# ai2cm/ace

Measured on AMD Instinct MI355X. Metric: rollout steps/sec (6-hourly forward steps of the 1-degree SFNO, whole job), higher is better.
Workload: dtype f32 (contractions with K>=32 on error-compensated fp16x3 MFMA, fp32 accumulate; DFT, norms, epilogues fp32; measured error vs fp64 below the fp32 CPU reference's); 1 GPU; ACE2-ERA5-shape 1deg SFNO rollout (BASELINE.json configs[1]): embed 384, 8 layers, dhconv, 44 in / 50 out channels, 180x360 legendre-gauss, lmax 180, mmax 181, B=1 member per GPU, random-init weights; members=1, members_per_gpu=1, graph=step, precision=f16x3, collective=none

## Files before the change

### ace_amd/build.py

```python

import concurrent.futures
import os
import shutil
import subprocess

HERE = os.path.dirname(os.path.abspath(__file__))
CSRC = os.path.join(HERE, "csrc")
OBJ = os.path.join(CSRC, "build")
LIB = os.path.join(HERE, "libace_sfno.so")
SOURCES = ["kernels.hip", "fft.hip", "strip.hip", "strip_fold.hip", "conv_ws.hip", "conv_wl.hip", "dhconv_strip.hip", "cln_mfma.hip", "physics.hip", "ocean_phys.hip", "masking.hip", "diag.hip", "hist.hip", "regress.hip", "calendar.hip", "healpix.hip", "latlon.hip", "capi.hip", "tables.cpp"]
HEADERS = ["kernels.h", "strip_common.h", "strip_pack.h", "ws_plan.h", "pack_frag.h", "dhconv_units.h", "tuning_guard.h", "small_fft.h", "tables.h", "diag_common.h", os.path.join("..", "..", "include", "ace_sfno.h")]
FLAGS = ["--offload-arch=gfx950", "-O3", "-std=c++17", "-fPIC"]


def _hipcc() -> str:
    for cand in (shutil.which("hipcc"), "/opt/rocm/bin/hipcc"):
        if cand and os.path.exists(cand):
            return cand
    raise RuntimeError("hipcc not found (need ROCm >= 7.0 to build libace_sfno.so)")


def _mtime(path: str) -> float:
    return os.path.getmtime(path) if os.path.exists(path) else 0.0


def _header_time() -> float:
    return max(_mtime(os.path.join(CSRC, h)) for h in HEADERS)


def source_sha256() -> str:
    import hashlib
    h = hashlib.sha256()
    for name in sorted(SOURCES + HEADERS):
        with open(os.path.join(CSRC, name), "rb") as f:
            h.update(name.encode() + b"\0" + f.read() + b"\0")
    h.update(" ".join(FLAGS).encode())
    return h.hexdigest()


def needs_build() -> bool:
    if not os.path.exists(LIB):
        return True
    t = os.path.getmtime(LIB)
    deps = [os.path.join(CSRC, s) for s in SOURCES + HEADERS]
    return any(os.path.exists(d) and os.path.getmtime(d) > t for d in deps)


def _compile(hipcc: str, src: str, obj: str, extra, verbose: bool) -> None:
    cmd = [hipcc] + FLAGS + list(extra) + ["-c", src, "-o", obj]
    if verbose:
        print(" ".join(cmd), flush=True)
    res = subprocess.run(cmd, capture_output=True, text=True)
    if res.returncode != 0:
        raise RuntimeError(f"hipcc failed on {src}:\n" + res.stdout + res.stderr)


def build(force: bool = False, verbose: bool = False, out: str = LIB, extra=(), objdir: str = OBJ) -> str:
    if out == LIB and extra:
        raise ValueError("the shipped library is built with the default flags only; a variant (extra flags) needs its own `out` and `objdir`")
    if extra and not any(f == "-DACE_MEASUREMENT_SWITCHES" for f in extra):
        extra = list(extra) + ["-DACE_MEASUREMENT_SWITCHES"]
    if not force and out == LIB and not needs_build():
        return LIB
    hipcc = _hipcc()
    os.makedirs(objdir, exist_ok=True)
    for stale in os.listdir(objdir):
        if stale.endswith(".o") and stale[:-2] not in SOURCES:
            os.remove(os.path.join(objdir, stale))
    ht = _header_time()
    jobs, objs = [], []
    for s in SOURCES:
        src = os.path.join(CSRC, s)
        obj = os.path.join(objdir, s + ".o")
        objs.append(obj)
        if force or _mtime(obj) < max(_mtime(src), ht):
            jobs.append((src, obj))
    with concurrent.futures.ThreadPoolExecutor(max_workers=max(1, min(len(jobs), os.cpu_count() or 1))) as ex:
        for f in [ex.submit(_compile, hipcc, src, obj, extra, verbose) for src, obj in jobs]:
            f.result()
    cmd = [hipcc, "--offload-arch=gfx950", "-shared", "-fPIC", "-o", out + ".tmp"] + objs
    if verbose:
        print(" ".join(cmd), flush=True)
    res = subprocess.run(cmd, capture_output=True, text=True)
    if res.returncode != 0:
        raise RuntimeError("link failed:\n" + res.stdout + res.stderr)
    os.replace(out + ".tmp", out)
    return out


if __name__ == "__main__":
    import sys

    print(build(force="--force" in sys.argv, verbose=True))
```

### ace_amd/csrc/conv_wl.hip

```cpp
#include <hip/hip_runtime.h>

#include <cstdint>

#include "strip_common.h"

namespace ace {
namespace {

#ifndef ACE_WL_WAVES
#define ACE_WL_WAVES 8
#endif
#ifndef ACE_WL_D
#define ACE_WL_D 4
#endif
#ifndef ACE_WL_ABL
#define ACE_WL_ABL 0
#endif
constexpr int WL_WAVES = ACE_WL_WAVES;
#ifdef ACE_X_TRACE
__device__ unsigned long long wl_wg_span[4096][3];
#define WG_STAMP(k) do { if (threadIdx.x == 0 && blockIdx.x < 4096) wl_wg_span[blockIdx.x][k] = __builtin_amdgcn_s_memtime(); } while (0)
#else
#define WG_STAMP(k) do { } while (0)
#endif
constexpr int WL_OOBV = 0x7fffff00;

template <int KS, int RT, int D, bool FOLD = false>
__global__ __launch_bounds__(64 * WL_WAVES) void conv_wl_kernel(ConvStripArgs p, int nslice, int groups_per_xcd, int tpx) {
    constexpr int FTB = FOLD ? (2 * 16 * KS + WL_WAVES * 32 * RT + 16) * 4 : 0;
    __shared__ __attribute__((aligned(16))) char smem[RT * KS * 2048 + 32 * RT * 4 + FTB];
    float* Pb = reinterpret_cast<float*>(smem + RT * KS * 2048);
    const int tid = threadIdx.x;
    const int lane = tid & 63;
    const int wave = __builtin_amdgcn_readfirstlane(tid >> 6);
    const int i = lane & 31, g = lane >> 5;

    const int per_xcd = nslice * groups_per_xcd;
    const int per_smp = 8 * per_xcd;
    const int smp = blockIdx.x / per_smp;
    const int bb = blockIdx.x % per_smp;
    const int xcd = bb & 7, w = bb >> 3;
    const int slice = w % nslice, grp = w / nslice;
    const int tiles_px = (p.HW + 31) / 32;
    const int x0 = xcd * tpx;
    const int x1 = x0 + tpx < tiles_px ? x0 + tpx : tiles_px;

    MT(0);
    WG_STAMP(0);
    const unsigned raw_x = slot_load(p.xslot + lane);
    const unsigned raw_a = (!FOLD && p.aslot) ? slot_load(p.aslot + lane) : 0u;
    const unsigned raw_c = p.cinb ? slot_load(p.cinb + lane) : 0u;

    float fscale = 1.f;
    if constexpr (FOLD) {
        static_assert(WL_WAVES == 8 && KS % 8 == 0, "fold: wave w takes the k-steps w, w + 8, ... of every row tile");
        float* Ta = Pb + 32 * RT;
        float* Tb = Ta + 16 * KS;
        float* Pd = Tb + 16 * KS;
        float* red = Pd + WL_WAVES * 32 * RT;
        const float* fa = p.fa + (long)smp * p.sfa;
        const float* fb = p.fb + (long)smp * p.sfa;
        float am = 0.f;
        for (int r = tid; r < 16 * KS; r += 64 * WL_WAVES) {
            const float av = fa[r];
            Ta[r] = av; Tb[r] = fb[r];
            am = fmaxf(am, fabsf(av));
        }
#pragma unroll
        for (int off = 32; off > 0; off >>= 1) am = fmaxf(am, __shfl_xor(am, off, 64));
        if (lane == 0) red[wave] = am;
        __syncthreads();
        am = red[0];
#pragma unroll
        for (int k = 1; k < WL_WAVES; ++k) am = fmaxf(am, red[k]);
        fscale = ldexpf(1.0f, pow2_exponent_for(p.wabs * am));
#pragma unroll
        for (int t = 0; t < RT; ++t) {
            const float* Wr = p.Wraw + (long)(32 * (slice * RT + t) + i) * p.ldw + 8 * g;
            float dot = 0.f;
#pragma unroll
            for (int jj = 0; jj < KS / 8; ++jj) {
                const int J = wave + 8 * jj;
                const f32x4 w0 = *reinterpret_cast<const f32x4*>(Wr + 16 * J), w1 = *reinterpret_cast<const f32x4*>(Wr + 16 * J + 4);
                const int col = 16 * J + 8 * g;
                const f32x4 a0 = *reinterpret_cast<const f32x4*>(Ta + col), a1 = *reinterpret_cast<const f32x4*>(Ta + col + 4);
                const f32x4 b0 = *reinterpret_cast<const f32x4*>(Tb + col), b1 = *reinterpret_cast<const f32x4*>(Tb + col + 4);
                half8 fh, fl;
#pragma unroll
                for (int e = 0; e < 8; ++e) {
                    const float wv = e < 4 ? w0[e & 3] : w1[e & 3];
                    dot = fmaf(wv, e < 4 ? b0[e & 3] : b1[e & 3], dot);
                    float x = wv * fscale;
                    x *= e < 4 ? a0[e & 3] : a1[e & 3];
                    x = __builtin_amdgcn_fmed3f(x, -65504.f, 65504.f);
                    const _Float16 hv = (_Float16)x;
                    fh[e] = hv;
                    fl[e] = (_Float16)(x - (float)hv);
                }
                *reinterpret_cast<half8*>(smem + (t * KS + J) * 2048 + lane * 16) = fh;
                *reinterpret_cast<half8*>(smem + (t * KS + J) * 2048 + 1024 + lane * 16) = fl;
            }
            dot += __shfl_xor(dot, 32, 64);
            if (g == 0) Pd[wave * (32 * RT) + 32 * t + i] = dot;
        }
        __syncthreads();
        if (tid < 32 * RT) {
            float acc = Pd[tid];
#pragma unroll
            for (int k = 1; k < WL_WAVES; ++k) acc += Pd[k * (32 * RT) + tid];
            Pb[tid] = p.bias[slice * 32 * RT + tid] + acc;
        }
    } else {
        const char* A = reinterpret_cast<const char*>(p.A + (long)smp * p.sA) + (long)slice * RT * KS * 2048;
        for (int o = tid * 16; o < RT * KS * 2048; o += 64 * WL_WAVES * 16)
            *reinterpret_cast<u32x4*>(smem + o) = *reinterpret_cast<const u32x4*>(A + o);
        const float* b = p.bias + (long)smp * p.sbias + slice * 32 * RT;
        if (tid < 32 * RT) Pb[tid] = b[tid];
    }
    const float xbound = wave_max_bits(raw_x);
    const float inv_x = ldexpf(1.0f, -pow2_exponent_for(xbound));
    const float inv_a = FOLD ? 1.0f / fscale : (p.aslot ? ldexpf(1.0f, -pow2_exponent_for(wave_max_bits(raw_a))) : 1.0f / p.ascale);
    const float s_acc = inv_x * inv_a;
    const float inb = p.cinb ? wave_max_bits(raw_c) : xbound;
    const float cbound = fmaf(p.cw, inb, p.cb);
    const float cscale = ldexpf(1.0f, pow2_exponent_for(cbound));
    if (tid == 0) atomicMax(p.cslot + (blockIdx.x & 63), __float_as_uint(cbound));
    __syncthreads();
    MT(1);
    int tev = 2;

    const _Float16* Xh = p.Xhi + (long)smp * p.sX;
    const _Float16* Xl = p.Xlo + (long)smp * p.sX;
    const int pbytes = p.M * p.HW * 2;
    const int xbytes = p.C * (int)p.ldn * 2;
    const auto rsXh = __builtin_amdgcn_make_buffer_rsrc(const_cast<_Float16*>(Xh), 0, xbytes, 0x00020000);
    const auto rsXl = __builtin_amdgcn_make_buffer_rsrc(const_cast<_Float16*>(Xl), 0, xbytes, 0x00020000);
    const auto rsH = __builtin_amdgcn_make_buffer_rsrc(p.Chi + (long)smp * p.sCp, 0, pbytes, 0x00020000);
    const auto rsL = __builtin_amdgcn_make_buffer_rsrc(p.Clo + (long)smp * p.sCp, 0, pbytes, 0x00020000);
    const char* aw = smem + lane * 16;

    f32x16 prev[RT];
#pragma unroll
    for (int t = 0; t < RT; ++t)
#pragma unroll
        for (int r = 0; r < 16; ++r) prev[t][r] = 0.f;
    int prev_vo = WL_OOBV;
    GeluStage gst = {0.f, 0.f, 0.f};
    unsigned hh[4] = {0u, 0u, 0u, 0u}, ll[4] = {0u, 0u, 0u, 0u};
    float bias_next = Pb[8 * g];
    auto chunk = [&](auto kc) {
        constexpr int k = decltype(kc)::value;
        constexpr int v = k / 4, ch = k % 4, t = v / 16, q = (v % 16) / 8, e = v % 8;
        if constexpr (ch == 0) {
            gelu_stage0(gst, fmaf(prev[t][8 * q + e], s_acc, bias_next));
            asm volatile("" : "+v"(gst.val), "+v"(gst.t));
        } else if constexpr (ch == 1) {
            gelu_stage1(gst);
            constexpr int vn = (v + 1) % (16 * RT);
            bias_next = Pb[32 * (vn / 16) + 16 * ((vn % 16) / 8) + 8 * g + vn % 8];
            asm volatile("" : "+v"(gst.q));
        } else if constexpr (ch == 2) {
            gst.val = gelu_stage2(gst);
            asm volatile("" : "+v"(gst.val));
        } else {
            split_put<e>(hh, ll, cscale, gst.val);
            if constexpr (e == 7) {
                const int soff = (4 * (slice * RT + t) + 2 * q) * p.HW * 16;
                __builtin_amdgcn_raw_buffer_store_b128(u32x4{hh[0], hh[1], hh[2], hh[3]}, rsH, prev_vo, soff, 0);
                __builtin_amdgcn_raw_buffer_store_b128(u32x4{ll[0], ll[1], ll[2], ll[3]}, rsL, prev_vo, soff, 0);
            }
        }
    };
    constexpr int NCH = 4 * 16 * RT;
    constexpr int NM = 9 * KS;
    static_assert(RT == 3 || RT == 2, "slot arithmetic below");
    constexpr int MPS = 3 * RT;
    auto slot = [&](auto mc) {
        constexpr int m = decltype(mc)::value;
        constexpr int NMT = MPS * KS;
        if constexpr (!(ACE_WL_ABL & 1)) static_for<(m * NCH) / NMT, ((m + 1) * NCH) / NMT>([&](auto kc) { chunk(kc); });
        __builtin_amdgcn_sched_barrier(0);
    };
    (void)NM;

    const int stride = WL_WAVES * groups_per_xcd;
    for (int tile = x0 + grp * WL_WAVES + wave; tile < x1; tile += stride) {
        MT(tev);
        int n = 32 * tile + i;
        const bool nok = n < p.HW;
        n = nok ? n : p.HW - 1;
        const int bvo = (g * (int)p.ldn + n) * 16;
        const int kstep = 2 * (int)p.ldn * 16;
        f32x16 acc[RT];
#pragma unroll
        for (int t = 0; t < RT; ++t)
#pragma unroll
            for (int r = 0; r < 16; ++r) acc[t][r] = 0.f;
        half8 bh[D], bl[D];
#pragma unroll
        for (int d = 0; d < D; ++d) {
            bh[d] = __builtin_bit_cast(half8, __builtin_amdgcn_raw_buffer_load_b128(rsXh, bvo, d * kstep, 0));
            bl[d] = __builtin_bit_cast(half8, __builtin_amdgcn_raw_buffer_load_b128(rsXl, bvo, d * kstep, 0));
        }
        half8 ah[2][RT], al[2][RT];
#pragma unroll
        for (int t = 0; t < RT; ++t) {
            ah[0][t] = *reinterpret_cast<const half8*>(aw + (t * KS) * 2048);
            al[0][t] = *reinterpret_cast<const half8*>(aw + (t * KS) * 2048 + 1024);
        }
        static_for<0, KS>([&](auto jc) {
            constexpr int j = decltype(jc)::value;
            const half8 ch = bh[j % D], cl = bl[j % D];
            if constexpr (j + 1 < KS) {
#pragma unroll
                for (int t = 0; t < RT; ++t) {
                    ah[(j + 1) & 1][t] = *reinterpret_cast<const half8*>(aw + (t * KS + j + 1) * 2048);
                    al[(j + 1) & 1][t] = *reinterpret_cast<const half8*>(aw + (t * KS + j + 1) * 2048 + 1024);
                }
            }
            __builtin_amdgcn_sched_barrier(0);
            static_for<0, RT>([&](auto tc) {
                constexpr int t = decltype(tc)::value;
                acc[t] = __builtin_amdgcn_mfma_f32_32x32x16_f16(al[j & 1][t], ch, acc[t], 0, 0, 0);
                slot(std::integral_constant<int, MPS * j + t>{});
            });
            static_for<0, RT>([&](auto tc) {
                constexpr int t = decltype(tc)::value;
                acc[t] = __builtin_amdgcn_mfma_f32_32x32x16_f16(ah[j & 1][t], cl, acc[t], 0, 0, 0);
                slot(std::integral_constant<int, MPS * j + RT + t>{});
            });
            static_for<0, RT>([&](auto tc) {
                constexpr int t = decltype(tc)::value;
                acc[t] = __builtin_amdgcn_mfma_f32_32x32x16_f16(ah[j & 1][t], ch, acc[t], 0, 0, 0);
                if constexpr (t == RT - 1 && j + D < KS && !(ACE_WL_ABL & 2)) {
                    bh[j % D] = __builtin_bit_cast(half8, __builtin_amdgcn_raw_buffer_load_b128(rsXh, bvo, (j + D) * kstep, 0));
                    bl[j % D] = __builtin_bit_cast(half8, __builtin_amdgcn_raw_buffer_load_b128(rsXl, bvo, (j + D) * kstep, 0));
                }
                slot(std::integral_constant<int, MPS * j + 2 * RT + t>{});
            });
        });
        MT(tev + 1);
        tev += 2;
#pragma unroll
        for (int t = 0; t < RT; ++t) {
            rows_to_kgroups(acc[t]);
            prev[t] = acc[t];
        }
        prev_vo = nok ? ((g * p.HW + 32 * tile + i) * 16) : WL_OOBV;
    }
    static_for<0, NCH>([&](auto kc) { chunk(kc); });
    MT(tev);
    WG_STAMP(1);
#ifdef ACE_X_TRACE
    if (threadIdx.x == 0 && blockIdx.x < 4096) {
        unsigned xcc;
        asm volatile("s_getreg_b32 %0, hwreg(HW_REG_XCC_ID)" : "=s"(xcc));
        wl_wg_span[blockIdx.x][2] = xcc & 0xf;
    }
#endif
}

template <int KS, int RT, int D, bool FOLD = false>
hipError_t launch_wl(const ConvStripArgs& a, hipStream_t s) {
    const int nslice = a.M / (32 * RT);
    int gpx = 32 / nslice;
    if (gpx < 1) gpx = 1;
    const int tiles_px = (int)((a.HW + 31) / 32);
    const int tpx = (tiles_px + 7) / 8;
    if (gpx * WL_WAVES > tpx) gpx = (tpx + WL_WAVES - 1) / WL_WAVES;
    dim3 grid((unsigned)(8 * nslice * gpx * a.nbatch)), block(64 * WL_WAVES);
    hipLaunchKernelGGL((conv_wl_kernel<KS, RT, D, FOLD>), grid, block, 0, s, a, nslice, gpx, tpx);
    return hipGetLastError();
}

}

#ifdef ACE_X_TRACE
extern "C" int ace_debug_trace(void* dst) { return (int)hipMemcpyFromSymbol(dst, HIP_SYMBOL(mlp_trace), sizeof(mlp_trace)); }
extern "C" int ace_debug_wg_spans(void* dst) { return (int)hipMemcpyFromSymbol(dst, HIP_SYMBOL(wl_wg_span), sizeof(wl_wg_span)); }
#endif

bool conv_wl_eligible(int K, int M, long HW) {
    if (K == 384) return M % 96 == 0 && M / 96 <= 32 && (long)M * HW * 2 < 0x7fffff00L;
    if (K == 512 || K == 256 || K == 128) return M % 64 == 0 && M / 64 <= 32 && (long)M * HW * 2 < 0x7fffff00L;
    return false;
}

hipError_t launch_conv_wl(const ConvStripArgs& a, hipStream_t s) {
    if (!conv_wl_eligible(a.C, a.M, a.HW) || !a.bias || !a.xslot || !(a.A || a.Wraw) || !a.Chi || !a.Clo || !a.cslot || a.R || a.part || a.Cf ||
        !(a.act == ACT_GELU || a.act == ACT_GELU_FAST))
        return hipErrorInvalidValue;
    if (a.Wraw) {
        if (!a.fa || !a.fb || (a.ldw & 3) != 0 || (reinterpret_cast<uintptr_t>(a.Wraw) & 15) != 0 || a.sbias != 0 || a.C != 384) return hipErrorInvalidValue;
        return launch_wl<24, 3, ACE_WL_D, true>(a, s);
    }
    switch (a.C) {
        case 512: return launch_wl<32, 2, 4>(a, s);
        case 384: return launch_wl<24, 3, ACE_WL_D>(a, s);
        case 256: return launch_wl<16, 2, 4>(a, s);
        case 128: return launch_wl<8, 2, 4>(a, s);
        default: return hipErrorInvalidValue;
    }
}

}
```

### ace_amd/csrc/strip_common.h

```cpp
#pragma once
#include <hip/hip_runtime.h>

#include <type_traits>

#include "kernels.h"

namespace ace {
namespace {

#define MDEV __device__ __forceinline__
#ifndef ACE_MLP_FDEPTH
#define ACE_MLP_FDEPTH 2
#endif
#ifndef ACE_MLP_ABL
#define ACE_MLP_ABL 0
#endif

typedef _Float16 half8 __attribute__((ext_vector_type(8)));
typedef float f32x16 __attribute__((ext_vector_type(16)));
typedef float f32x4 __attribute__((ext_vector_type(4)));
typedef unsigned u32x4 __attribute__((ext_vector_type(4)));
typedef __attribute__((address_space(3))) char* lds_cptr;

MDEV unsigned slot_load(const unsigned* p) { return __hip_atomic_load(p, __ATOMIC_RELAXED, __HIP_MEMORY_SCOPE_AGENT); }
MDEV int pow2_exponent_for(float mx) {
    int e = 0;
    if (mx > 0.f && mx < 3.0e38f) { (void)frexpf(mx, &e); e = 12 - e; }
    return e > 100 ? 100 : (e < -100 ? -100 : e);
}
MDEV float wave_max_bits(unsigned raw) {
    float mx = __uint_as_float(raw);
#pragma unroll
    for (int off = 32; off > 0; off >>= 1) mx = fmaxf(mx, __shfl_xor(mx, off, 64));
    return __uint_as_float(__builtin_amdgcn_readfirstlane(__float_as_uint(mx)));
}
MDEV void glds16(const void* gsrc, const char* lds_dst_uniform) {
    const unsigned addr = __builtin_amdgcn_readfirstlane((unsigned)(size_t)(lds_cptr)lds_dst_uniform);
    asm volatile("s_mov_b32 m0, %1\n\ts_nop 0\n\tglobal_load_lds_dwordx4 %0, off"
                 :
                 : "v"(gsrc), "s"(addr)
                 : "memory", "m0");
}
MDEV void glds16s(const void* sbase_uniform, unsigned lane_off, const char* lds_dst_uniform) {
    const unsigned addr = __builtin_amdgcn_readfirstlane((unsigned)(size_t)(lds_cptr)lds_dst_uniform);
    asm volatile("s_mov_b32 m0, %2\n\ts_nop 0\n\tglobal_load_lds_dwordx4 %0, %1"
                 :
                 : "v"(lane_off), "s"(sbase_uniform), "s"(addr)
                 : "memory", "m0");
}
MDEV unsigned lds_addr_of(const char* p) { return __builtin_amdgcn_readfirstlane((unsigned)(size_t)(lds_cptr)p); }
MDEV void glds16a(const void* sbase_uniform, unsigned lane_off, unsigned lds_addr_uniform) {
    asm volatile("s_mov_b32 m0, %2\n\ts_nop 0\n\tglobal_load_lds_dwordx4 %0, %1"
                 :
                 : "v"(lane_off), "s"(sbase_uniform), "s"(lds_addr_uniform)
                 : "memory", "m0");
}
MDEV float fast_erf(float x) {
    const float t = fminf(fabsf(x), 4.0f);
    float q = -1.150086973e-05f;
    q = fmaf(q, t, 1.518900972e-04f);
    q = fmaf(q, t, -8.436889620e-04f);
    q = fmaf(q, t, 2.264559502e-03f);
    q = fmaf(q, t, -7.151089812e-05f);
    q = fmaf(q, t, -2.773463540e-02f);
    q = fmaf(q, t, 1.483123451e-01f);
    q = fmaf(q, t, 9.184418917e-01f);
    q = fmaf(q, t, 1.627907395e+00f);
    q = q * t;
    return copysignf(1.0f - __builtin_amdgcn_exp2f(-q), x);
}
struct GeluStage { float val, t, q; };
MDEV void gelu_stage0(GeluStage& g, float val) {
    g.val = val;
    g.t = fminf(fabsf(val), 5.65685424949238f);
}
MDEV void gelu_stage1(GeluStage& g) {
    float q = -5.082714551e-07f;
    q = fmaf(q, g.t, 9.493131074e-06f);
    q = fmaf(q, g.t, -7.457227184e-05f);
    q = fmaf(q, g.t, 2.830699377e-04f);
    q = fmaf(q, g.t, -1.264146067e-05f);
    q = fmaf(q, g.t, -6.933658849e-03f);
    q = fmaf(q, g.t, 5.243633315e-02f);
    q = fmaf(q, g.t, 4.592209458e-01f);
    q = fmaf(q, g.t, 1.151104331e+00f);
    g.q = q;
}
MDEV float gelu_stage2(const GeluStage& g) {
    const float q = g.q * g.t;
    const float s = g.val + fabsf(g.val);
    return 0.5f * fmaf(-g.t, __builtin_amdgcn_exp2f(-q), s);
}

template <int E>
MDEV void split_put(unsigned (&H)[4], unsigned (&L)[4], const float cs, const float v) {
    constexpr int d = E >> 1;
    if constexpr ((E & 1) == 0) {
        asm volatile("v_fma_mixlo_f16 %0, %2, %3, 0\n\tv_fma_mixlo_f16 %1, %2, %3, -%0 op_sel_hi:[0,0,1]" : "+v"(H[d]), "+v"(L[d]) : "v"(cs), "v"(v));
    } else {
        unsigned tmp;
        asm volatile("v_fma_mixlo_f16 %2, %3, %4, 0\n\tv_fma_mixhi_f16 %0, %3, %4, 0\n\tv_fma_mixhi_f16 %1, %3, %4, -%2 op_sel_hi:[0,0,1]"
                     : "+v"(H[d]), "+v"(L[d]), "=&v"(tmp)
                     : "v"(cs), "v"(v));
    }
}

template <int ACT>
MDEV float act_fn(float v) {
    if (ACT == ACT_GELU_FAST || ACT == ACT_GELU) { GeluStage g; gelu_stage0(g, v); gelu_stage1(g); return gelu_stage2(g); }
    if (ACT == ACT_RELU) return v > 0.f ? v : 0.f;
    if (ACT == ACT_SILU) return v / (1.0f + expf(-v));
    return v;
}

MDEV void rows_to_kgroups(f32x16& v) {
#pragma unroll
    for (int hq = 0; hq < 2; ++hq)
#pragma unroll
        for (int e = 0; e < 4; ++e) {
            const auto sw = __builtin_amdgcn_permlane32_swap(__float_as_uint(v[8 * hq + e]), __float_as_uint(v[8 * hq + 4 + e]), false, false);
            v[8 * hq + e] = __uint_as_float(sw[0]);
            v[8 * hq + 4 + e] = __uint_as_float(sw[1]);
        }
}

#ifdef ACE_X_TRACE
__device__ unsigned long long mlp_trace[512];
#define MT(ev) do { if (blockIdx.x == ACE_X_TRACE && threadIdx.x == 0 && (ev) < 512) mlp_trace[ev] = __builtin_amdgcn_s_memtime(); } while (0)
#else
#define MT(ev) do { } while (0)
#endif

template <int I0, int I1, class F>
MDEV void static_for(F&& f);

struct Frag { half8 h, l; };
template <int OFF>
MDEV void frag_issue(Frag& f, unsigned lds_addr) {
    asm volatile("ds_read_b128 %0, %2 offset:%3\n\tds_read_b128 %1, %2 offset:%4"
                 : "=&v"(f.h), "=&v"(f.l)
                 : "v"(lds_addr), "n"(OFF), "n"(OFF + 1024));
}
template <int N>
MDEV void frag_wait(Frag& f) {
    asm volatile("s_waitcnt lgkmcnt(%2)" : "+v"(f.h), "+v"(f.l) : "n"(N));
}
template <int NS, int DEPTH, class F>
MDEV void pipelined_steps(unsigned lds_addr, F&& body) {
    Frag fr[DEPTH + 1];
    static_for<0, (DEPTH < NS ? DEPTH : NS)>([&](auto ss) {
        constexpr int s0 = decltype(ss)::value;
        frag_issue<s0 * 2048>(fr[s0 % (DEPTH + 1)], lds_addr);
    });
    static_for<0, NS>([&](auto ss) {
        constexpr int st = decltype(ss)::value;
        if constexpr (st + DEPTH < NS) frag_issue<(st + DEPTH) * 2048>(fr[(st + DEPTH) % (DEPTH + 1)], lds_addr);
        constexpr int newer = (NS - 1 - st) < DEPTH ? (NS - 1 - st) : DEPTH;
        frag_wait<2 * newer>(fr[st % (DEPTH + 1)]);
        body(ss, fr[st % (DEPTH + 1)]);
    });
}

template <int NS, class F>
MDEV void pipelined_pairs(unsigned lds_addr, F&& body) {
    static_assert(NS % 2 == 0, "units of two k-steps");
    constexpr int NU = NS / 2;
    Frag fr[2][2];
#if ACE_MLP_ABL & 2
    for (int a = 0; a < 2; ++a) for (int b = 0; b < 2; ++b) { asm volatile("" : "=v"(fr[a][b].h), "=v"(fr[a][b].l)); }
    static_for<0, NU>([&](auto uu) { constexpr int u = decltype(uu)::value; body(uu, fr[u % 2][0], fr[u % 2][1]); });
    return;
#endif
    frag_issue<0>(fr[0][0], lds_addr);
    frag_issue<2048>(fr[0][1], lds_addr);
    static_for<0, NU>([&](auto uu) {
        constexpr int u = decltype(uu)::value;
        if constexpr (u + 1 < NU) {
            frag_issue<(2 * u + 2) * 2048>(fr[(u + 1) % 2][0], lds_addr);
            frag_issue<(2 * u + 3) * 2048>(fr[(u + 1) % 2][1], lds_addr);
        }
        constexpr int newer = u + 1 < NU ? 4 : 0;
        asm volatile("s_waitcnt lgkmcnt(%4)"
                     : "+v"(fr[u % 2][0].h), "+v"(fr[u % 2][0].l), "+v"(fr[u % 2][1].h), "+v"(fr[u % 2][1].l)
                     : "n"(newer));
        body(uu, fr[u % 2][0], fr[u % 2][1]);
    });
}

template <int I0, int I1, class F>
MDEV void static_for(F&& f) {
    if constexpr (I0 < I1) {
        f(std::integral_constant<int, I0>{});
        static_for<I0 + 1, I1>(f);
    }
}


}
}
```

### ace_amd/csrc/tuning_guard.h

```cpp
#pragma once
#if !defined(ACE_MEASUREMENT_SWITCHES)
#if defined(ACE_WL_ABL) || defined(ACE_WL_D) || defined(ACE_WL_WAVES) || defined(ACE_WS_ABL) || defined(ACE_WS_ACC2) || defined(ACE_WS_FD4) || \
    defined(ACE_WS_FINE) || defined(ACE_WS_HOLD4) || defined(ACE_WS_VSPAN) || defined(ACE_WS_REARLY) || defined(ACE_WS_MINMAX) || defined(ACE_FFT_ABL) || defined(ACE_FFT_FWD_WAVES) || defined(ACE_FFT_FWD_PLN_WAVES) ||            \
    defined(ACE_FFT_INV_ROWS) || defined(ACE_FFT_INV_WAVES) || defined(ACE_FFT_QROWS) || defined(ACE_FFT_ROWS) || defined(ACE_FFT_XCD) ||       \
    defined(ACE_FFT_XCD_INV) || defined(ACE_G4_PIN) || defined(ACE_EXP_NOLDSREAD) || defined(ACE_EXP_NOBARRIER) || defined(ACE_EXP_NOGLOBAL) || \
    defined(ACE_EXP_NOLDSWRITE) || defined(ACE_G3_W128_PCT) || defined(ACE_G4_PFD) || defined(ACE_G4_REGEPI) || defined(ACE_G4_RTOUCH) ||       \
    defined(ACE_GEMM2_BK) || defined(ACE_LB) || defined(ACE_PF) || defined(ACE_MLP_ABL) || defined(ACE_MLP_FDEPTH) || defined(ACE_X_TRACE) ||    \
    defined(ACE_DH_TRACE) || defined(ACE_DH_TRACE_WG) || defined(ACE_DH_PB) || defined(ACE_DH_WGS) || defined(ACE_DH_STRIPS) || defined(ACE_DH_ORDER) || defined(ACE_LF_TRACE) || defined(ACE_DEBUG_WS)
#error "tuning / ablation / trace macro set without -DACE_MEASUREMENT_SWITCHES: the shipped library is built with the defaults only (tools/mkvar.sh)"
#endif
#endif
```

Before: 185.7 steps/s.

## Switch conv_wl main loop from 32x32x16 to 16x16x32 MFMA tiles

Adds a default-on path in the conv_wl kernel that computes each 32x32 output tile as four 16x16 sub-tiles using the 16x16x32 f16 MFMA, with new lane/offset maps for the A reads from LDS and the B loads from global. The accumulators are permuted back into the old k-group register layout with permlane16_swap, so the epilogue stays unchanged. The aim is to use the MFMA shape with higher issue throughput or better latency hiding on gfx950. In exchange it issues four times as many MFMA instructions, changes the load pattern and register use, and adds a cross-lane shuffle per tile.

```diff
diff --git a/ace_amd/build.py b/ace_amd/build.py
--- a/ace_amd/build.py
+++ b/ace_amd/build.py
@@ -9,7 +9,7 @@
 OBJ = os.path.join(CSRC, "build")
 LIB = os.path.join(HERE, "libace_sfno.so")
 SOURCES = ["kernels.hip", "fft.hip", "strip.hip", "strip_fold.hip", "conv_ws.hip", "conv_wl.hip", "dhconv_strip.hip", "cln_mfma.hip", "physics.hip", "ocean_phys.hip", "masking.hip", "diag.hip", "hist.hip", "regress.hip", "calendar.hip", "healpix.hip", "latlon.hip", "capi.hip", "tables.cpp"]
-HEADERS = ["kernels.h", "strip_common.h", "strip_pack.h", "ws_plan.h", "pack_frag.h", "dhconv_units.h", "tuning_guard.h", "small_fft.h", "tables.h", "diag_common.h", os.path.join("..", "..", "include", "ace_sfno.h")]
+HEADERS = ["kernels.h", "strip_common.h", "mfma16_map.h", "strip_pack.h", "ws_plan.h", "pack_frag.h", "dhconv_units.h", "tuning_guard.h", "small_fft.h", "tables.h", "diag_common.h", os.path.join("..", "..", "include", "ace_sfno.h")]
 FLAGS = ["--offload-arch=gfx950", "-O3", "-std=c++17", "-fPIC"]
 
 
diff --git a/ace_amd/csrc/conv_wl.hip b/ace_amd/csrc/conv_wl.hip
--- a/ace_amd/csrc/conv_wl.hip
+++ b/ace_amd/csrc/conv_wl.hip
@@ -15,6 +15,9 @@
 #endif
 #ifndef ACE_WL_ABL
 #define ACE_WL_ABL 0
+#endif
+#ifndef ACE_WL_SHAPE16
+#define ACE_WL_SHAPE16 1
 #endif
 constexpr int WL_WAVES = ACE_WL_WAVES;
 #ifdef ACE_X_TRACE
@@ -25,7 +28,7 @@
 #endif
 constexpr int WL_OOBV = 0x7fffff00;
 
-template <int KS, int RT, int D, bool FOLD = false>
+template <int KS, int RT, int D, bool FOLD = false, bool S16 = (ACE_WL_SHAPE16 != 0)>
 __global__ __launch_bounds__(64 * WL_WAVES) void conv_wl_kernel(ConvStripArgs p, int nslice, int groups_per_xcd, int tpx) {
     constexpr int FTB = FOLD ? (2 * 16 * KS + WL_WAVES * 32 * RT + 16) * 4 : 0;
     __shared__ __attribute__((aligned(16))) char smem[RT * KS * 2048 + 32 * RT * 4 + FTB];
@@ -174,7 +177,7 @@
     constexpr int NCH = 4 * 16 * RT;
     constexpr int NM = 9 * KS;
     static_assert(RT == 3 || RT == 2, "slot arithmetic below");
-    constexpr int MPS = 3 * RT;
+    constexpr int MPS = S16 ? 6 * RT : 3 * RT;
     auto slot = [&](auto mc) {
         constexpr int m = decltype(mc)::value;
         constexpr int NMT = MPS * KS;
@@ -189,62 +192,126 @@
         int n = 32 * tile + i;
         const bool nok = n < p.HW;
         n = nok ? n : p.HW - 1;
-        const int bvo = (g * (int)p.ldn + n) * 16;
-        const int kstep = 2 * (int)p.ldn * 16;
-        f32x16 acc[RT];
-#pragma unroll
-        for (int t = 0; t < RT; ++t)
-#pragma unroll
-            for (int r = 0; r < 16; ++r) acc[t][r] = 0.f;
-        half8 bh[D], bl[D];
-#pragma unroll
-        for (int d = 0; d < D; ++d) {
-            bh[d] = __builtin_bit_cast(half8, __builtin_amdgcn_raw_buffer_load_b128(rsXh, bvo, d * kstep, 0));
-            bl[d] = __builtin_bit_cast(half8, __builtin_amdgcn_raw_buffer_load_b128(rsXl, bvo, d * kstep, 0));
-        }
-        half8 ah[2][RT], al[2][RT];
-#pragma unroll
-        for (int t = 0; t < RT; ++t) {
-            ah[0][t] = *reinterpret_cast<const half8*>(aw + (t * KS) * 2048);
-            al[0][t] = *reinterpret_cast<const half8*>(aw + (t * KS) * 2048 + 1024);
-        }
-        static_for<0, KS>([&](auto jc) {
-            constexpr int j = decltype(jc)::value;
-            const half8 ch = bh[j % D], cl = bl[j % D];
-            if constexpr (j + 1 < KS) {
-#pragma unroll
-                for (int t = 0; t < RT; ++t) {
-                    ah[(j + 1) & 1][t] = *reinterpret_cast<const half8*>(aw + (t * KS + j + 1) * 2048);
-                    al[(j + 1) & 1][t] = *reinterpret_cast<const half8*>(aw + (t * KS + j + 1) * 2048 + 1024);
+        if constexpr (S16) {
+            static_assert(D % 2 == 0 && KS % 2 == 0, "k32-steps");
+            constexpr int DJ = D / 2, NJ = KS / 2;
+            int bvo[2];
+#pragma unroll
+            for (int ph = 0; ph < 2; ++ph) {
+                int np = 32 * tile + m16::b_pixel(ph, lane);
+                np = np < p.HW ? np : p.HW - 1;
+                bvo[ph] = (m16::b_kgroup(0, lane) * (int)p.ldn + np) * 16;
+            }
+            const int kstep = m16::b_kgroup(1, 0) * (int)p.ldn * 16;
+            f32x4 acc[RT][2][2];
+#pragma unroll
+            for (int t = 0; t < RT; ++t)
+#pragma unroll
+                for (int r = 0; r < 16; ++r) acc[t][r >> 3][(r >> 2) & 1][r & 3] = 0.f;
+            half8 bh[DJ][2], bl[DJ][2];
+#pragma unroll
+            for (int d = 0; d < DJ; ++d)
+#pragma unroll
+                for (int ph = 0; ph < 2; ++ph) {
+                    bh[d][ph] = __builtin_bit_cast(half8, __builtin_amdgcn_raw_buffer_load_b128(rsXh, bvo[ph], d * kstep, 0));
+                    bl[d][ph] = __builtin_bit_cast(half8, __builtin_amdgcn_raw_buffer_load_b128(rsXl, bvo[ph], d * kstep, 0));
                 }
-            }
-            __builtin_amdgcn_sched_barrier(0);
-            static_for<0, RT>([&](auto tc) {
-                constexpr int t = decltype(tc)::value;
-                acc[t] = __builtin_amdgcn_mfma_f32_32x32x16_f16(al[j & 1][t], ch, acc[t], 0, 0, 0);
-                slot(std::integral_constant<int, MPS * j + t>{});
+            const char* aw16[2] = {smem + m16::a_lane_byte(0, lane), smem + m16::a_lane_byte(1, lane)};
+            auto a_read = [&](auto hc, half8 (&dh)[RT], half8 (&dl)[RT]) {
+                constexpr int hs = decltype(hc)::value, J = hs >> 1, a = hs & 1;
+                static_for<0, RT>([&](auto kc) {
+                    constexpr int rt = a * RT + decltype(kc)::value;
+                    const char* src = aw16[rt & 1] + m16::a_row_tile32(rt) * KS * 2048 + J * m16::A_STEP_BYTES;
+                    dh[decltype(kc)::value] = *reinterpret_cast<const half8*>(src);
+                    dl[decltype(kc)::value] = *reinterpret_cast<const half8*>(src + m16::A_LO_BYTES);
+                });
+            };
+            half8 ah[2][RT], al[2][RT];
+            a_read(std::integral_constant<int, 0>{}, ah[0], al[0]);
+            static_for<0, 2 * NJ>([&](auto hc) {
+                constexpr int hs = decltype(hc)::value, J = hs >> 1, a = hs & 1;
+                if constexpr (hs + 1 < 2 * NJ) a_read(std::integral_constant<int, hs + 1>{}, ah[(hs + 1) & 1], al[(hs + 1) & 1]);
+                __builtin_amdgcn_sched_barrier(0);
+                static_for<0, 3>([&](auto pc) {
+                    constexpr int pr = decltype(pc)::value;
+                    static_for<0, 2 * RT>([&](auto kc) {
+                        constexpr int k = decltype(kc)::value, x = k >> 1, ph = k & 1, rt = a * RT + x;
+                        const half8 av = pr == 0 ? al[hs & 1][x] : ah[hs & 1][x];
+                        const half8 bv = pr == 1 ? bl[J % DJ][ph] : bh[J % DJ][ph];
+                        acc[rt >> 1][rt & 1][ph] = __builtin_amdgcn_mfma_f32_16x16x32_f16(av, bv, acc[rt >> 1][rt & 1][ph], 0, 0, 0);
+                        if constexpr (a == 1 && pr == 2 && k == 2 * RT - 1 && J + DJ < NJ && !(ACE_WL_ABL & 2)) {
+#pragma unroll
+                            for (int q = 0; q < 2; ++q) {
+                                bh[J % DJ][q] = __builtin_bit_cast(half8, __builtin_amdgcn_raw_buffer_load_b128(rsXh, bvo[q], (J + DJ) * kstep, 0));
+                                bl[J % DJ][q] = __builtin_bit_cast(half8, __builtin_amdgcn_raw_buffer_load_b128(rsXl, bvo[q], (J + DJ) * kstep, 0));
+                            }
+                        }
+                        slot(std::integral_constant<int, MPS * hs + 2 * RT * pr + k>{});
+                    });
+                });
             });
-            static_for<0, RT>([&](auto tc) {
-                constexpr int t = decltype(tc)::value;
-                acc[t] = __builtin_amdgcn_mfma_f32_32x32x16_f16(ah[j & 1][t], cl, acc[t], 0, 0, 0);
-                slot(std::integral_constant<int, MPS * j + RT + t>{});
+            MT(tev + 1);
+            tev += 2;
+#pragma unroll
+            for (int t = 0; t < RT; ++t) prev[t] = tiles16_to_kgroups(acc[t]);
+        } else {
+            const int bvo = (g * (int)p.ldn + n) * 16;
+            const int kstep = 2 * (int)p.ldn * 16;
+            f32x16 acc[RT];
+    #pragma unroll
+            for (int t = 0; t < RT; ++t)
+    #pragma unroll
+                for (int r = 0; r < 16; ++r) acc[t][r] = 0.f;
+            half8 bh[D], bl[D];
+    #pragma unroll
+            for (int d = 0; d < D; ++d) {
+                bh[d] = __builtin_bit_cast(half8, __builtin_amdgcn_raw_buffer_load_b128(rsXh, bvo, d * kstep, 0));
+                bl[d] = __builtin_bit_cast(half8, __builtin_amdgcn_raw_buffer_load_b128(rsXl, bvo, d * kstep, 0));
+            }
+            half8 ah[2][RT], al[2][RT];
+    #pragma unroll
+            for (int t = 0; t < RT; ++t) {
+                ah[0][t] = *reinterpret_cast<const half8*>(aw + (t * KS) * 2048);
+                al[0][t] = *reinterpret_cast<const half8*>(aw + (t * KS) * 2048 + 1024);
+            }
+            static_for<0, KS>([&](auto jc) {
+                constexpr int j = decltype(jc)::value;
+                const half8 ch = bh[j % D], cl = bl[j % D];
+                if constexpr (j + 1 < KS) {
+    #pragma unroll
+                    for (int t = 0; t < RT; ++t) {
+                        ah[(j + 1) & 1][t] = *reinterpret_cast<const half8*>(aw + (t * KS + j + 1) * 2048);
+                        al[(j + 1) & 1][t] = *reinterpret_cast<const half8*>(aw + (t * KS + j + 1) * 2048 + 1024);
+                    }
+                }
+                __builtin_amdgcn_sched_barrier(0);
+                static_for<0, RT>([&](auto tc) {
+                    constexpr int t = decltype(tc)::value;
+                    acc[t] = __builtin_amdgcn_mfma_f32_32x32x16_f16(al[j & 1][t], ch, acc[t], 0, 0, 0);
+                    slot(std::integral_constant<int, MPS * j + t>{});
+                });
+                static_for<0, RT>([&](auto tc) {
+                    constexpr int t = decltype(tc)::value;
+                    acc[t] = __builtin_amdgcn_mfma_f32_32x32x16_f16(ah[j & 1][t], cl, acc[t], 0, 0, 0);
+                    slot(std::integral_constant<int, MPS * j + RT + t>{});
+                });
+                static_for<0, RT>([&](auto tc) {
+                    constexpr int t = decltype(tc)::value;
+                    acc[t] = __builtin_amdgcn_mfma_f32_32x32x16_f16(ah[j & 1][t], ch, acc[t], 0, 0, 0);
+                    if constexpr (t == RT - 1 && j + D < KS && !(ACE_WL_ABL & 2)) {
+                        bh[j % D] = __builtin_bit_cast(half8, __builtin_amdgcn_raw_buffer_load_b128(rsXh, bvo, (j + D) * kstep, 0));
+                        bl[j % D] = __builtin_bit_cast(half8, __builtin_amdgcn_raw_buffer_load_b128(rsXl, bvo, (j + D) * kstep, 0));
+                    }
+                    slot(std::integral_constant<int, MPS * j + 2 * RT + t>{});
+                });
             });
-            static_for<0, RT>([&](auto tc) {
-                constexpr int t = decltype(tc)::value;
-                acc[t] = __builtin_amdgcn_mfma_f32_32x32x16_f16(ah[j & 1][t], ch, acc[t], 0, 0, 0);
-                if constexpr (t == RT - 1 && j + D < KS && !(ACE_WL_ABL & 2)) {
-                    bh[j % D] = __builtin_bit_cast(half8, __builtin_amdgcn_raw_buffer_load_b128(rsXh, bvo, (j + D) * kstep, 0));
-                    bl[j % D] = __builtin_bit_cast(half8, __builtin_amdgcn_raw_buffer_load_b128(rsXl, bvo, (j + D) * kstep, 0));
-                }
-                slot(std::integral_constant<int, MPS * j + 2 * RT + t>{});
-            });
-        });
-        MT(tev + 1);
-        tev += 2;
-#pragma unroll
-        for (int t = 0; t < RT; ++t) {
-            rows_to_kgroups(acc[t]);
-            prev[t] = acc[t];
+            MT(tev + 1);
+            tev += 2;
+    #pragma unroll
+            for (int t = 0; t < RT; ++t) {
+                rows_to_kgroups(acc[t]);
+                prev[t] = acc[t];
+            }
         }
         prev_vo = nok ? ((g * p.HW + 32 * tile + i) * 16) : WL_OOBV;
     }
diff --git a/ace_amd/csrc/mfma16_map.h b/ace_amd/csrc/mfma16_map.h
--- /dev/null
+++ b/ace_amd/csrc/mfma16_map.h
@@ -0,0 +1,32 @@
+#pragma once
+
+#if defined(__HIPCC__)
+#define M16_FN __host__ __device__ constexpr inline
+#else
+#define M16_FN constexpr inline
+#endif
+
+namespace ace {
+namespace m16 {
+
+M16_FN int a_row_tile32(int rt) { return rt >> 1; }
+M16_FN int a_kstep16(int J, int l) { return 2 * J + (l >> 5); }
+M16_FN int a_src_lane(int rt, int l) { return 16 * (rt & 1) + (l & 15) + 32 * ((l >> 4) & 1); }
+M16_FN int a_lane_byte(int rt, int l) { return (l >> 5) * 2048 + a_src_lane(rt, l) * 16; }
+constexpr int A_STEP_BYTES = 4096, A_LO_BYTES = 1024;
+
+M16_FN int b_kgroup(int J, int l) { return 4 * J + (l >> 4); }
+M16_FN int b_pixel(int ph, int l) { return 16 * ph + (l & 15); }
+
+M16_FN int d_row(int l, int r) { return 4 * (l >> 4) + r; }
+M16_FN int d_pixel(int ph, int l) { return 16 * ph + (l & 15); }
+M16_FN int swap_from_lane(bool is_src, int l) {
+    const bool odd_row = (l >> 4) & 1;
+    return is_src ? (odd_row ? -1 : l + 16) : (odd_row ? l - 16 : -1);
+}
+M16_FN int kg_register(int rt, int ph, int r) { return 8 * (rt & 1) + 4 * ph + r; }
+M16_FN int kg_row(int rt, int ph, int r, int l) { return 16 * (rt & 1) + 8 * (l >> 5) + 4 * ph + r; }
+M16_FN int kg_pixel(int l) { return l & 31; }
+
+}
+}
diff --git a/ace_amd/csrc/strip_common.h b/ace_amd/csrc/strip_common.h
--- a/ace_amd/csrc/strip_common.h
+++ b/ace_amd/csrc/strip_common.h
@@ -4,6 +4,7 @@
 #include <type_traits>
 
 #include "kernels.h"
+#include "mfma16_map.h"
 
 namespace ace {
 namespace {
@@ -161,6 +162,19 @@
     });
 }
 
+MDEV f32x16 tiles16_to_kgroups(f32x4 (&a)[2][2]) {
+    f32x16 v;
+#pragma unroll
+    for (int rt = 0; rt < 2; ++rt)
+#pragma unroll
+        for (int r = 0; r < 4; ++r) {
+            const auto sw = __builtin_amdgcn_permlane16_swap(__float_as_uint(a[rt][0][r]), __float_as_uint(a[rt][1][r]), false, false);
+            v[m16::kg_register(rt, 0, r)] = __uint_as_float(sw[0]);
+            v[m16::kg_register(rt, 1, r)] = __uint_as_float(sw[1]);
+        }
+    return v;
+}
+
 template <int NS, class F>
 MDEV void pipelined_pairs(unsigned lds_addr, F&& body) {
     static_assert(NS % 2 == 0, "units of two k-steps");
diff --git a/ace_amd/csrc/tuning_guard.h b/ace_amd/csrc/tuning_guard.h
--- a/ace_amd/csrc/tuning_guard.h
+++ b/ace_amd/csrc/tuning_guard.h
@@ -6,7 +6,8 @@
     defined(ACE_FFT_XCD_INV) || defined(ACE_G4_PIN) || defined(ACE_EXP_NOLDSREAD) || defined(ACE_EXP_NOBARRIER) || defined(ACE_EXP_NOGLOBAL) || \
     defined(ACE_EXP_NOLDSWRITE) || defined(ACE_G3_W128_PCT) || defined(ACE_G4_PFD) || defined(ACE_G4_REGEPI) || defined(ACE_G4_RTOUCH) ||       \
     defined(ACE_GEMM2_BK) || defined(ACE_LB) || defined(ACE_PF) || defined(ACE_MLP_ABL) || defined(ACE_MLP_FDEPTH) || defined(ACE_X_TRACE) ||    \
-    defined(ACE_DH_TRACE) || defined(ACE_DH_TRACE_WG) || defined(ACE_DH_PB) || defined(ACE_DH_WGS) || defined(ACE_DH_STRIPS) || defined(ACE_DH_ORDER) || defined(ACE_LF_TRACE) || defined(ACE_DEBUG_WS)
+    defined(ACE_DH_TRACE) || defined(ACE_DH_TRACE_WG) || defined(ACE_DH_PB) || defined(ACE_DH_WGS) || defined(ACE_DH_STRIPS) || defined(ACE_DH_ORDER) || defined(ACE_LF_TRACE) || defined(ACE_DEBUG_WS) || \
+    defined(ACE_WL_SHAPE16)
 #error "tuning / ablation / trace macro set without -DACE_MEASUREMENT_SWITCHES: the shipped library is built with the defaults only (tools/mkvar.sh)"
 #endif
 #endif
```

After: 185.8 steps/s (median of 2 runs). No clear change (+0.1%).
